# tianyili2017/HEVC-Complexity-Reduction

Measured on AMD Instinct MI355X. Metric: CTUs/sec (ETH-CNN inference), higher is better.
Workload: dtype f32; 1 GPU; All-Intra 3840x2160 QP32, 50 frames synthetic YUV; width=3840, height=2160, frames_per_gpu=50, qp=32, ranks=1, devices_visible=1, rank0_device=0, one_rank_per_device=True, device=AMD Radeon Graphics (gfx950:sramecc+:xnack-, 256 CUs), host NUMA node 1

## Files before the change

### hevc-complexity-reduction_amd/csrc/ethcnn_context.cpp

```cpp
#include "ethcnn_ctx.h"

static thread_local std::string g_create_err;

int set_err(ethcnn_ctx* c, int code, const char* fmt, ...) {
    char buf[512];
    va_list ap;
    va_start(ap, fmt);
    std::vsnprintf(buf, sizeof buf, fmt, ap);
    va_end(ap);
    if (c) c->err = buf; else g_create_err = buf;
    return code;
}

extern "C" const char* ethcnn_version(void) { return "ethcnn-mi355x 0.1 (gfx950)"; }

extern "C" const char* ethcnn_last_error(const ethcnn_ctx* ctx) {
    return ctx ? ctx->err.c_str() : g_create_err.c_str();
}

int ensure_side_streams(ethcnn_ctx* c) {
    hipStream_t* ss[] = {&c->copy_in, &c->copy_out, &c->s_tile};
    for (hipStream_t* s : ss)
        if (!*s) HIPCHK(c, hipStreamCreateWithFlags(s, hipStreamNonBlocking));
    return 0;
}

static void free_workspace(ethcnn_ctx* c) {
    Workspace& w = c->ws;
    void* ptrs[] = {w.featb, w.xs, w.xm, w.xl, w.feat, w.h1, w.h2, w.logits, w.raw, w.flags, c->xs1, c->xm1, c->xl1, c->h1_1, c->flags1};
    for (void* p : ptrs)
        if (p) (void)hipFree(p);
    w = Workspace();
    c->xs1 = c->xm1 = c->xl1 = nullptr;
    c->h1_1 = nullptr;
    c->flags1 = nullptr;
}

Workspace ws_view(const ethcnn_ctx* c, int p) {
// ... 188 lines not shown
    {
        std::vector<std::thread> th;
        for (ethcnn_ctx* p : c->peers)
            if (p) th.emplace_back([p] { ethcnn_destroy(p); });
        for (auto& t : th) t.join();
        c->peers.clear();
    }
    (void)hipSetDevice(c->device);
    for (const auto& r : c->pinned) (void)hipHostFree(const_cast<char*>(r.first));
    delete c->pool;
    if (c->dw_arena) (void)hipFree(c->dw_arena);
    if (c->dw_fast) (void)hipFree(c->dw_fast);
    if (c->dw_trunk16) (void)hipFree(c->dw_trunk16);
    if (c->dw_heads16) (void)hipFree(c->dw_heads16);
    {
        void* lp[] = {c->d_lstm, c->d_vec, c->d_state[0], c->d_state[1], c->d_lprobs, c->d_lgate, c->d_ssync, c->seq_vec, c->seq_probs, c->narrow_buf, c->d_compare};
        for (void* p : lp)
            if (p) (void)hipFree(p);
    }
    {
        hipEvent_t evs[] = {c->e_tile[0], c->e_tile[1], c->e_trunk[0], c->e_trunk[1], c->e_main, c->e_fc1[0], c->e_fc1[1], c->e_band[0], c->e_band[1], c->e_band[2], c->e_band[3]};
        for (hipEvent_t e : evs)
            if (e) (void)hipEventDestroy(e);
    }
    hipStream_t streams[] = {c->stream, c->copy_in, c->copy_out, c->s_tile};
    for (hipStream_t st : streams)
        if (st) (void)hipStreamDestroy(st);
    delete c;
}

extern "C" int ethcnn_get_startup_times(const ethcnn_ctx* c, double* runtime_init_ms, double* create_ms) {
// ... 182 lines not shown
```

### hevc-complexity-reduction_amd/csrc/ethcnn_ctx.h

```cpp
#pragma once
#include <hip/hip_runtime.h>
#if defined(__SSE2__)
#include <emmintrin.h>
#endif
#include <sched.h>
#include <sys/stat.h>
#include <unistd.h>

#include <algorithm>
#include <cerrno>
#include <cstdarg>
#include <cstdio>
#include <cstdlib>
#include <cstring>
#include <atomic>
#include <chrono>
#include <condition_variable>
#include <functional>
#include <mutex>
#include <string>
#include <thread>
#include <vector>

#include "ethcnn_kernels.h"
// ... 120 lines not shown
    float* seq_vec = nullptr;
    float* seq_probs = nullptr;
    size_t seq_vec_cap = 0, seq_probs_cap = 0;
    int seq_chunk = 0;
    ethcnn_source_format src_fmt{8, 420};
    uint8_t* narrow_buf = nullptr;
    size_t narrow_cap = 0;
    int narrow_chunk = 0;
    std::vector<uint8_t> narrow_host;

    Workspace ws;
    uint4 *xs1 = nullptr, *xm1 = nullptr, *xl1 = nullptr;
    float* h1_1 = nullptr;
    int* flags1 = nullptr;
    hipStream_t s_tile = nullptr;
    hipEvent_t e_tile[2] = {}, e_trunk[2] = {}, e_main = nullptr;
    hipEvent_t e_fc1[2] = {};
    int tile_after_fc1 = 0;
    hipEvent_t e_band[4] = {};
    int* d_lgate = nullptr;
    int lgate_chunks = 0;
    bool lgate_clean = false;
    int lgate_n = -1;
    int lstm_epoch = 0;
    int lstm_one_launch = 1;
    int tile_blocks = 256;
    unsigned pass_idx = 0;
    int last_parity = 0;
    int small_launch = 1;
    bool luma_over_pcie = false;
// ... 144 lines not shown
```

### hevc-complexity-reduction_amd/csrc/ethcnn_dense.hip

```cpp
#include <hip/hip_runtime.h>

#include <cstdlib>

#include "ethcnn_kernels.h"
#include "ethcnn_fc1_regs.h"
#include "ethcnn_fc1_tile.h"

namespace ethcnn {

template <int MS, int NS, int WM, int NSUB, bool GROUP, int NST = 3>
__global__ __launch_bounds__(64 * WM) void k_fc1_p3(const float* __restrict__ feat, const float* __restrict__ Wimg,
                                                    const float* __restrict__ bias, float* __restrict__ out, int M) {
    __shared__ __attribute__((aligned(16))) float smem[Fc1Shape<MS, NS, WM, NSUB, NST>::LDS_FLOATS];
    fc1_tile<MS, NS, WM, NSUB, GROUP, NST>(smem, feat, Wimg, bias, out, M, blockIdx.x);
}

#ifdef FC1_STAMPS
__device__ unsigned long long g_fc1_stamps[1 << 14][2];
__device__ __forceinline__ void fc1_stamp(int slot) {
    unsigned long long t;
    asm volatile("s_memrealtime %0\n\ts_waitcnt lgkmcnt(0)" : "=s"(t)::"memory");
    if (threadIdx.x == 0) g_fc1_stamps[blockIdx.x & 0x3fff][slot] = t;
}
#define FC1_STAMP(i) fc1_stamp(i)
#else
#define FC1_STAMP(i)
#endif

#ifndef FC1_BULK_NST
#define FC1_BULK_NST 3
#endif
template <int NS, int WM, int NSUB>
__global__ __launch_bounds__(64 * WM) void k_fc1_bulk(const float* __restrict__ feat, const float* __restrict__ Wimg,
                                                      const float* __restrict__ bias, float* __restrict__ out, int m_main,
                                                      int m_total, unsigned rem_blocks) {
    __shared__ __attribute__((aligned(16))) float smem[Fc1Shape<2, NS, WM, NSUB, FC1_BULK_NST>::LDS_FLOATS];
    FC1_STAMP(0);
    if (blockIdx.x < rem_blocks)
        fc1_tile<1, NS, WM, NSUB, true, FC1_BULK_NST>(smem, feat + (size_t)(m_main / 16) * kNFeat * 16, Wimg, bias, out + (size_t)m_main * kNVec,
                                           m_total - m_main, blockIdx.x);
    else
        fc1_tile<2, NS, WM, NSUB, true, FC1_BULK_NST>(smem, feat, Wimg, bias, out, m_main, blockIdx.x - rem_blocks);
    FC1_STAMP(1);
}

template <int MS, int NS, int WM, int NSUB, bool GROUP = false, int NST = 3>
static void launch_fc1_p3(const float* feat, const float* wimg, const float* bias, float* out, int M, hipStream_t s) {
    constexpr int BM = 16 * MS * WM, NSPLIT = kNVec / (16 * NS);
    const int mtiles = (M + BM - 1) / BM;
    const int blocks = GROUP ? ((mtiles + 7) / 8) * 8 * NSPLIT : mtiles * NSPLIT;
    hipLaunchKernelGGL((k_fc1_p3<MS, NS, WM, NSUB, GROUP, NST>), dim3(blocks), dim3(64 * WM), 0, s, feat, wimg, bias, out, M);
}

template <int NS, int D>
__global__ __launch_bounds__(256) void k_fc1_regs(const float* __restrict__ feat, const float* __restrict__ wlane,
                                                  const float* __restrict__ bias, float* __restrict__ out, int M) {
    int mt, nb;
    fc1_block_to_tile<kNVec / (16 * NS), true>(blockIdx.x, mt, nb);
    if (mt * 64 >= M) return;
    fc1_tile_regs<NS, D, false>(feat, wlane, bias, out, M, mt, nb);
}
template <int NS, int D>
static void launch_fc1_regs(const float* feat, const float* wlane, const float* bias, float* out, int M, hipStream_t s) {
    constexpr int NSPLIT = kNVec / (16 * NS);
    const int mtiles = (M + 63) / 64;
    hipLaunchKernelGGL((k_fc1_regs<NS, D>), dim3(((mtiles + 7) / 8) * 8 * NSPLIT), dim3(256), 0, s, feat, wlane, bias, out, M);
// ... 20 lines not shown
    double tbest = 1e30;
    for (const Shape& sh : shapes) {
        const int blocks = ((n + sh.bm - 1) / sh.bm) * sh.nsplit;
        const double t = sh.a + sh.b * ((blocks + 255) / 256);
        if (t < tbest) { tbest = t; best = sh.variant; }
    }
    return best;
}

static void launch_fc1_rows(int variant, const Workspace& ws, const DeviceWeights& w, int row0, int rows, float* out,
                            hipStream_t s) {
    const float* feat = ws.feat + (size_t)(row0 / 16) * kNFeat * 16;
    float* o = out + (size_t)row0 * kNVec;
    switch (variant) {
        default:
            launch_fc1_p3<2, 7, 4, 1, true>(feat, w.fc1_img112, w.fc1_b, o, rows, s);
            break;
        case 1:
            launch_fc1_p3<1, 7, 4, 1, true>(feat, w.fc1_img112, w.fc1_b, o, rows, s);
            break;
        case 2:
            launch_fc1_p3<1, 4, 4, 2, true>(feat, w.fc1_img64, w.fc1_b, o, rows, s);
            break;
        case 3:
            launch_fc1_p3<1, 2, 4, 2, true>(feat, w.fc1_img32, w.fc1_b, o, rows, s);
            break;
        case 4:
            launch_fc1_p3<1, 1, 4, 4, true>(feat, w.fc1_img16, w.fc1_b, o, rows, s);
            break;
        case 5:
            launch_fc1_p3<1, 2, 4, 4, true>(feat, w.fc1_img32, w.fc1_b, o, rows, s);
            break;
        case 6:
            launch_fc1_p3<1, 2, 2, 4, true>(feat, w.fc1_img32, w.fc1_b, o, rows, s);
            break;
        case 7: launch_fc1_regs<1, 16>(feat, w.fc1_lane16, w.fc1_b, o, rows, s); break;
        case 8: launch_fc1_regs<2, 10>(feat, w.fc1_lane16, w.fc1_b, o, rows, s); break;
        case 9: launch_fc1_regs<4, 6>(feat, w.fc1_lane16, w.fc1_b, o, rows, s); break;
        case 10: launch_fc1_p3<2, 7, 4, 1, false>(feat, w.fc1_img112, w.fc1_b, o, rows, s); break;
        case 11: launch_fc1_p3<1, 7, 4, 1, false>(feat, w.fc1_img112, w.fc1_b, o, rows, s); break;
        case 12: launch_fc1_p3<1, 4, 4, 2, false>(feat, w.fc1_img64, w.fc1_b, o, rows, s); break;
    }
}

void launch_fc1(const Workspace& ws, const DeviceWeights& w, int n, float* out, hipStream_t s) {
    const int variant = fc1_variant();
    if (variant >= 100) {
        const int bt = ((n / 128) * 4 / 256) * 256 / 4;
        if (bt > 0) launch_fc1_rows(0, ws, w, 0, bt * 128, out, s);
        if (n > bt * 128) launch_fc1_rows(variant - 100, ws, w, bt * 128, n - bt * 128, out, s);
        return;
    }
    if (variant >= 0 && variant != 20 && variant != 30) {
        launch_fc1_rows(variant, ws, w, 0, n, out, s);
        return;
    }
    if (variant == 20) {
        launch_fc1_rows(fc1_short_variant(n), ws, w, 0, n, out, s);
        return;
    }
    const int big_tiles = ((n / 128) * 4 / 256) * 256 / 4;
    const int row0 = big_tiles * 128;
    if (big_tiles >= 3 * 192 && n > row0 && fc1_variant() != 30) {
        const int rem_tiles = (n - row0 + 63) / 64;
        const unsigned rem_blocks = (unsigned)((rem_tiles + 7) / 8) * 8 * 4;
        const unsigned main_blocks = (unsigned)((big_tiles + 7) / 8) * 8 * 4;
        hipLaunchKernelGGL((k_fc1_bulk<7, 4, 1>), dim3(rem_blocks + main_blocks), dim3(256), 0, s, ws.feat, w.fc1_img112, w.fc1_b, out,
                           row0, n, rem_blocks);
        return;
    }
    if (big_tiles > 0) launch_fc1_rows(0, ws, w, 0, row0, out, s);
    if (n > row0) launch_fc1_rows(fc1_short_variant(n - row0), ws, w, row0, n - row0, out, s);
}

}
```

### hevc-complexity-reduction_amd/csrc/ethcnn_fc1_tile.h

```cpp
#pragma once
#include <hip/hip_runtime.h>

#include "ethcnn_kernels.h"

namespace ethcnn {

typedef float f32x4 __attribute__((ext_vector_type(4)));
typedef __attribute__((address_space(3))) void lds_void;
typedef const __attribute__((address_space(1))) void glb_void;
#ifndef MFMA16
#define MFMA16(a, b, c) __builtin_amdgcn_mfma_f32_16x16x4f32((a), (b), (c), 0, 0, 0)
#endif
constexpr int kAuxSc1 = 16;

template <int N>
__device__ __forceinline__ void vm_wait() { asm volatile("s_waitcnt vmcnt(%0)" ::"n"(N) : "memory"); }
template <int ISSUE, int MAXK>
__device__ __forceinline__ void vm_wait_groups(int keep) {
    if constexpr (MAXK == 0) {
        vm_wait<0>();
    } else {
        if (keep >= MAXK) vm_wait<MAXK * ISSUE>();
        else vm_wait_groups<ISSUE, MAXK - 1>(keep);
    }
// ... 6 lines not shown
    static constexpr int LDS_FLOATS = NST * STAGE;
};

template <int NSPLIT, bool GROUP>
__device__ __forceinline__ void fc1_block_to_tile(unsigned bid, int& mt, int& nb) {
    if (GROUP) {
        const int xcd = bid & 7, slot = bid >> 3;
        nb = slot % NSPLIT;
        mt = (slot / NSPLIT) * 8 + xcd;
    } else {
        nb = (int)(bid % NSPLIT);
        mt = (int)(bid / NSPLIT);
    }
}

template <int MS, int NS, int WM, int NSUB, int NST, bool COHERENT = false, bool A_SC1 = false>
__device__ __forceinline__ void fc1_tile_at(float* __restrict__ smem, const float* __restrict__ feat, const float* __restrict__ Wimg,
                                            const float* __restrict__ bias, float* __restrict__ out, int M, const int mt, const int nb) {
    constexpr int BK = 16 * NSUB, BN = 16 * NS, BM = 16 * MS * WM;
    constexpr int NK = kNFeat / BK;
    constexpr int B_FLOATS = BK * BN;
    constexpr bool COLSWZ = (BN % 32 == 0);
    constexpr int B_INST = B_FLOATS / 256;
    constexpr int B_PER = (B_INST + WM - 1) / WM;
    constexpr int A_PER = NSUB * MS;
    constexpr int ISSUE = B_PER + A_PER;
    constexpr int A_FLOATS = WM * A_PER * 256;
    constexpr int STAGE = B_FLOATS + A_FLOATS;
    constexpr int DIST = NST - 1;
    static_assert(NK % NST == 0 && NK >= NST, "K chunks must come in whole rounds of the stage ring");
    static_assert(DIST * ISSUE <= 63, "vmcnt is a 6-bit counter");
    static_assert(STAGE == Fc1Shape<MS, NS, WM, NSUB, NST>::STAGE, "LDS budget of the shape");

    const int lane = threadIdx.x & 63, wv = threadIdx.x >> 6;
    const int col = lane & 15, g = lane >> 4;
    const int m0 = mt * BM + wv * 16 * MS;
    const int n0 = nb * BN;

    f32x4 acc[MS][NS];
#pragma unroll
    for (int i = 0; i < MS; ++i)
#pragma unroll
        for (int j = 0; j < NS; ++j) acc[i][j] = (f32x4){0.f, 0.f, 0.f, 0.f};

    const int ngroups = (M + 15) >> 4;
    const unsigned wvu = __builtin_amdgcn_readfirstlane(wv);
    const unsigned lane16 = (unsigned)lane * 16u;
    const int mg0 = __builtin_amdgcn_readfirstlane(m0 >> 4);
    const float* a_base[MS];
#pragma unroll
    for (int i = 0; i < MS; ++i) a_base[i] = feat + (size_t)min(mg0 + i, ngroups - 1) * (kNFeat / 4) * 64;
    const float* b_base[B_PER];
    unsigned b_dst[B_PER];
#pragma unroll
    for (int i = 0; i < B_PER; ++i) {
        const unsigned piece = min(wvu + i * WM, (unsigned)(B_INST - 1));
        b_base[i] = Wimg + (size_t)nb * NK * B_FLOATS + (size_t)piece * 256;
        b_dst[i] = piece * 1024u;
    }
    int bcol[NS];
#pragma unroll
    for (int j = 0; j < NS; ++j) bcol[j] = (j * 16 + col) ^ (COLSWZ ? ((g & 1) << 4) : 0);
    int brow[4];
#pragma unroll
    for (int e = 0; e < 4; ++e) brow[e] = (COLSWZ ? e : (e ^ (g & 1))) * BN;
    float* a_lds = smem + B_FLOATS + wv * A_PER * 256;

    const unsigned lds_base = __builtin_amdgcn_readfirstlane((unsigned)(size_t)(lds_void*)smem);
    const unsigned a_dst0 = lds_base + 4u * (B_FLOATS + wvu * A_PER * 256);
#define P3_DMA(sbase, lds_byte_addr)                                                                   \
    {                                                                                                  \
        unsigned keep_;                                                                                \
        asm volatile("s_mov_b32 %0, m0\n\ts_mov_b32 m0, %3\n\ts_nop 0\n\tglobal_load_lds_dwordx4 %1, %2\n\ts_mov_b32 m0, %0" \
                     : "=&s"(keep_) : "v"(lane16), "s"(sbase), "s"(lds_byte_addr) : "memory");          \
    }
#define P3_DMA_SC1(sbase, lds_byte_addr)                                                               \
    {                                                                                                  \
        unsigned keep_;                                                                                \
        asm volatile("s_mov_b32 %0, m0\n\ts_mov_b32 m0, %3\n\ts_nop 0\n\tglobal_load_lds_dwordx4 %1, %2 sc1\n\ts_mov_b32 m0, %0" \
                     : "=&s"(keep_) : "v"(lane16), "s"(sbase), "s"(lds_byte_addr) : "memory");          \
    }
#define P3_ISSUE(kc, st)                                                                               \
    {                                                                                                  \
        _Pragma("unroll") for (int i = 0; i < B_PER; ++i)                                              \
            P3_DMA(b_base[i] + (size_t)(kc) * B_FLOATS, lds_base + 4u * (st) * STAGE + b_dst[i]);      \
        _Pragma("unroll") for (int u = 0; u < NSUB; ++u)                                               \
            _Pragma("unroll") for (int i = 0; i < MS; ++i) {                                           \
                if (A_SC1) P3_DMA_SC1(a_base[i] + ((size_t)(kc) * NSUB + u) * 256,                     \
                                      a_dst0 + 4u * ((st) * STAGE + (u * MS + i) * 256))               \
                else P3_DMA(a_base[i] + ((size_t)(kc) * NSUB + u) * 256,                               \
                            a_dst0 + 4u * ((st) * STAGE + (u * MS + i) * 256))                         \
            }                                                                                          \
    }
#define P3_COMPUTE(st)                                                                                 \
    {                                                                                                  \
        _Pragma("unroll") for (int u = 0; u < NSUB; ++u) {                                             \
            float4 av[MS];                                                                             \
            _Pragma("unroll") for (int i = 0; i < MS; ++i)                                             \
                av[i] = *reinterpret_cast<const float4*>(a_lds + (st) * STAGE + (u * MS + i) * 256 + lane * 4); \
            const float* bs = smem + (st) * STAGE + (16 * u + 4 * g) * BN;                             \
            _Pragma("unroll") for (int e = 0; e < 4; ++e) {                                            \
                float b[NS];                                                                           \
                _Pragma("unroll") for (int j = 0; j < NS; ++j) b[j] = bs[brow[e] + bcol[j]];           \
                _Pragma("unroll") for (int i = 0; i < MS; ++i) {                                       \
                    const float a = (e == 0) ? av[i].x : (e == 1) ? av[i].y : (e == 2) ? av[i].z : av[i].w; \
                    _Pragma("unroll") for (int j = 0; j < NS; ++j) acc[i][j] = MFMA16(a, b[j], acc[i][j]); \
                }                                                                                      \
            }                                                                                          \
        }                                                                                              \
    }
#define P3_STEP(kc, st)                                                                                \
    {                                                                                                  \
        if ((kc) + DIST < NK) { P3_ISSUE((kc) + DIST, ((st) + DIST) % NST); }                          \
        P3_COMPUTE(st);                                                                                \
        vm_wait_groups<ISSUE, DIST - 1>(NK - 2 - (kc));                                                \
        asm volatile("s_waitcnt lgkmcnt(0)" ::: "memory");                                             \
        __builtin_amdgcn_s_barrier();                                                                  \
    }

    __builtin_amdgcn_s_setprio(2);
#pragma unroll
// ... 14 lines not shown
    const int lane_out = ((m0 + 4 * g) * kNVec + col) * 4;
#pragma unroll
    for (int j = 0; j < NS; ++j) {
        const float bv = bias[n0 + j * 16 + col];
#pragma unroll
        for (int i = 0; i < MS; ++i)
#pragma unroll
            for (int r = 0; r < 4; ++r) {
                const float h = acc[i][j][r] + bv;
                __builtin_amdgcn_raw_buffer_store_b32(__builtin_bit_cast(unsigned, fmaxf(0.2f * h, h)), rO,
                                                      lane_out + (i * 16 + r) * kNVec * 4, (n0 + j * 16) * 4, COHERENT ? kAuxSc1 : 0);
            }
    }
}

template <int MS, int NS, int WM, int NSUB, bool GROUP, int NST>
__device__ __forceinline__ void fc1_tile(float* __restrict__ smem, const float* __restrict__ feat, const float* __restrict__ Wimg,
                                         const float* __restrict__ bias, float* __restrict__ out, int M, const unsigned bid) {
    int mt, nb;
    fc1_block_to_tile<kNVec / (16 * NS), GROUP>(bid, mt, nb);
    if (mt * (16 * MS * WM) >= M) return;
    fc1_tile_at<MS, NS, WM, NSUB, NST>(smem, feat, Wimg, bias, out, M, mt, nb);
}


}
```

### hevc-complexity-reduction_amd/csrc/ethcnn_kernels.h

```cpp
#pragma once
#include <hip/hip_runtime.h>

#include "ethcnn_spec.h"

namespace ethcnn {

struct Workspace {
    int cap = 0;
    uint4* xs = nullptr;
    uint4* xm = nullptr;
    uint4* xl = nullptr;
    float* feat = nullptr;
    uint16_t* featb = nullptr;
    float* h1 = nullptr;
    float* h2 = nullptr;
    float* logits = nullptr;
    float* raw = nullptr;
    int* flags = nullptr;
    int flags_cap = 0;
};

struct FrameGeom {
    int width, height;
    long pitch, frame_stride;
    int cw, ch, nctu;
};

void launch_tile(const uint8_t* d_luma, const FrameGeom& g, long ctu0, int n, const Workspace& ws, int n_flags,
                 hipStream_t s, int max_blocks = 0, const unsigned* wait_rows = nullptr, unsigned wait_seq = 0, unsigned* gave_up = nullptr);
void launch_trunk(const Workspace& ws, const DeviceWeights& w, int n, bool resi, hipStream_t s, int fc1_plan = 0);
void launch_trunk_f16(const Workspace& ws, const DeviceWeights& w, int n, hipStream_t s);
void launch_trunk_f16_foldall(const uint8_t* d_luma, const FrameGeom& g, long ctu0, int n, const Workspace& ws, const DeviceWeights& w, int n_flags,
                              hipStream_t s);
void launch_fc1(const Workspace& ws, const DeviceWeights& w, int n, float* out, hipStream_t s);
void launch_fc1_fast(const Workspace& ws, const DeviceWeights& w, int n, float* out, int plan, hipStream_t s, int cus = 256);
void launch_heads(const Workspace& ws, const DeviceWeights& w, int n, float qn, int nctu_per_frame,
                  long ctu0, float thr1, float thr2, float* d_probs, hipStream_t s);
void launch_heads_f16(const Workspace& ws, const DeviceWeights& w, int n, float qn, int nctu_per_frame, long ctu0, float thr1, float thr2,
                      float* d_probs, hipStream_t s);
#ifdef ETHCNN_FULL_FENCE
#define ETHCNN_HANDOFF_RELEASE() asm volatile("buffer_wbl2 sc1\n\ts_waitcnt vmcnt(0) lgkmcnt(0)" ::: "memory")
#define ETHCNN_HANDOFF_ACQUIRE() asm volatile("buffer_inv sc1" ::: "memory")
#else
#define ETHCNN_HANDOFF_RELEASE() asm volatile("s_waitcnt vmcnt(0)" ::: "memory")
// ... 53 lines not shown
```

### hevc-complexity-reduction_amd/csrc/ethcnn_kernels.hip

```cpp
#include <hip/hip_runtime.h>

#include <cstdlib>

#include "ethcnn_kernels.h"

namespace ethcnn {

int chunks_per_frame(int nctu) { return (nctu + kSubBatch - 1) / kSubBatch; }


__global__ __launch_bounds__(256) void k5_gate(float* __restrict__ probs, const int* __restrict__ flags, int N,
                                               GateIndex gi, float thr2) {
    const int idx = blockIdx.x * 256 + threadIdx.x;
    const int i = idx / kNOut, j = idx % kNOut;
    if (i >= N || j == 0) return;
    const int chunk = gate_chunk(gi, i);
    const bool open32 = flags[2 * chunk] != 0;
    const bool open16 = open32 ? (flags[2 * chunk + 1] != 0) : (0.0f > thr2);
    if (j < 5 ? !open32 : !open16) probs[(size_t)i * kNOut + j] = 0.0f;
}

void launch_gate(const Workspace& ws, int n, int nctu, long ctu0, float thr2, float* d_probs, hipStream_t s) {
    const long total = (long)n * kNOut;
    hipLaunchKernelGGL(k5_gate, dim3((unsigned)((total + 255) / 256)), dim3(256), 0, s, d_probs, ws.flags, n,
                       make_gate_index(nctu, ctu0), thr2);
}

typedef float f32x4_cal __attribute__((ext_vector_type(4)));
__global__ __launch_bounds__(256) void k_mfma_rate(int iters, float* sink) {
    f32x4_cal acc[4] = {{0.f, 0.f, 0.f, 0.f}, {0.f, 0.f, 0.f, 0.f}, {0.f, 0.f, 0.f, 0.f}, {0.f, 0.f, 0.f, 0.f}};
    const float a = 1.0f + threadIdx.x * 1e-7f, b = 0.999f;
    for (int i = 0; i < iters; ++i) {
#pragma unroll
        for (int u = 0; u < 8; ++u)
#pragma unroll
            for (int j = 0; j < 4; ++j) acc[j] = __builtin_amdgcn_mfma_f32_16x16x4f32(a, b, acc[j], 0, 0, 0);
    }
    const float s = acc[0][0] + acc[1][1] + acc[2][2] + acc[3][3];
    if (s == 123.456f) *sink = s;
}
// ... 6 lines not shown
```

### hevc-complexity-reduction_amd/csrc/ethcnn_model.cpp

```cpp
#include "ethcnn_ctx.h"

static int upload_weights(ethcnn_ctx* c) {
    HIPCHK(c, hipSetDevice(c->device));
    std::vector<size_t> sizes = {(size_t)3 * kTrunkWFrags * 64, (size_t)3 * kTrunkBFrags * 64,
                                 (size_t)kNFeat * kNVec, (size_t)kNVec};
    for (int h = 0; h < 3; ++h) { sizes.push_back((size_t)(kN1[h] + 1) * kN2[h]); sizes.push_back((size_t)kN2[h]); }
    for (int h = 0; h < 3; ++h) { sizes.push_back((size_t)(kN2[h] + 1) * kN3[h]); sizes.push_back((size_t)kN3[h]); }
    sizes.push_back((size_t)kNFeat * kNVec);
    sizes.push_back((size_t)kNFeat * kNVec);
    sizes.push_back((size_t)kNFeat * kNVec);
    sizes.push_back((size_t)kNFeat * kNVec);
    for (int h = 0; h < 3; ++h) sizes.push_back((size_t)kN1[h] * kN2[h]);
    std::vector<size_t> offs;
    size_t total = 0;
    for (size_t s : sizes) { offs.push_back(total); total += (s + 63) / 64 * 64; }
    std::vector<float> host(total, 0.0f);
    const float* blob = c->blob.data();
    pack_trunk_fragments(blob, host.data() + offs[0], host.data() + offs[1]);
    {
        std::vector<float> wcat((size_t)kNFeat * kNVec);
        pack_fc1(blob, wcat.data(), host.data() + offs[3]);
        pack_fc1_image(wcat.data(), 112, 16, host.data() + offs[2]);
        pack_fc1_image(wcat.data(), 64, 32, host.data() + offs[16]);
        pack_fc1_image(wcat.data(), 32, 32, host.data() + offs[17]);
        pack_fc1_image(wcat.data(), 16, 32, host.data() + offs[18]);
        pack_fc1_lane_image(wcat.data(), host.data() + offs[19]);
    }
    for (int h = 0; h < 3; ++h) {
        std::memcpy(host.data() + offs[4 + 2 * h], blob + kOffFc2W[h], sizes[4 + 2 * h] * 4);
        std::memcpy(host.data() + offs[5 + 2 * h], blob + kOffFc2B[h], sizes[5 + 2 * h] * 4);
        std::memcpy(host.data() + offs[10 + 2 * h], blob + kOffFc3W[h], sizes[10 + 2 * h] * 4);
        std::memcpy(host.data() + offs[11 + 2 * h], blob + kOffFc3B[h], sizes[11 + 2 * h] * 4);
        pack_fc2_lane_image(blob + kOffFc2W[h], kN1[h], kN2[h], host.data() + offs[20 + h]);
    }
    if (!c->dw_arena) HIPCHK(c, hipMalloc((void**)&c->dw_arena, total * 4));
    HIPCHK(c, hipDeviceSynchronize());
    HIPCHK(c, hipMemcpy(c->dw_arena, host.data(), total * 4, hipMemcpyHostToDevice));
    DeviceWeights& d = c->dw;
    d.trunk_w = c->dw_arena + offs[0];
    d.trunk_b = c->dw_arena + offs[1];
    d.fc1_img112 = c->dw_arena + offs[2];
    d.fc1_img64 = c->dw_arena + offs[16];
    d.fc1_img32 = c->dw_arena + offs[17];
    d.fc1_img16 = c->dw_arena + offs[18];
    d.fc1_lane16 = c->dw_arena + offs[19];
    for (int h = 0; h < 3; ++h) d.fc2_lane[h] = c->dw_arena + offs[20 + h];
    d.fc1_b = c->dw_arena + offs[3];
    for (int h = 0; h < 3; ++h) {
        d.fc2_w[h] = c->dw_arena + offs[4 + 2 * h];
        d.fc2_b[h] = c->dw_arena + offs[5 + 2 * h];
        d.fc3_w[h] = c->dw_arena + offs[10 + 2 * h];
        d.fc3_b[h] = c->dw_arena + offs[11 + 2 * h];
    }
    d.fc1_fast = nullptr;
    d.trunk16_w = nullptr;
    d.heads16_w = nullptr;
    d.trunk16_c = nullptr;
    c->guard_state[2] = c->guard_state[3] = 0;
    ++c->weights_gen;
    c->have_weights = true;
    return ETHCNN_OK;
// ... 280 lines not shown
```

### hevc-complexity-reduction_amd/csrc/ethcnn_pass.cpp

```cpp
#include "ethcnn_ctx.h"

int make_geom(ethcnn_ctx* c, int w, int h, ptrdiff_t pitch, ptrdiff_t fstride, FrameGeom* g) {
    if (w <= 0 || h <= 0) return set_err(c, ETHCNN_ERR_ARG, "bad frame size %dx%d", w, h);
    if (pitch < w) return set_err(c, ETHCNN_ERR_ARG, "pitch %td < width %d", pitch, w);
    g->width = w;
    g->height = h;
    g->pitch = (long)pitch;
    g->frame_stride = (long)fstride;
    g->cw = (w + 63) / 64;
    g->ch = (h + 63) / 64;
    g->nctu = g->cw * g->ch;
    return 0;
}

unsigned done_arm(ethcnn_ctx* c) {
    if (!c->done_sync || !c->h_done) return 0;
    if (++c->done_seq == 0) ++c->done_seq;
    return c->done_seq;
}
hipError_t stream_sync(ethcnn_ctx* c) {
    const unsigned seq = c->done_armed;
    c->done_armed = 0;
    if (seq) {
        const auto t0 = std::chrono::steady_clock::now();
// ... 49 lines not shown
    const int cpf = chunks_per_frame(g.nctu);
    const long nchunks = (ctu0 + n - 1) / g.nctu * cpf + ((ctu0 + n - 1) % g.nctu) / kSubBatch + 1 -
                         (ctu0 / g.nctu * cpf + (ctu0 % g.nctu) / kSubBatch);
    c->done_armed = 0;
    const bool takes_small = c->small_launch && n < kPipelineMinCtus && small_pass_ok(d_luma, g, n);
    int rc = (c->fc1_plan && !takes_small) ? ensure_fast_weights(c, c->fc1_plan) : 0;
    if (rc) return rc;
    rc = ensure_workspace(c, n, (int)nchunks);
    if (rc) return rc;
    const float qn = (float)qp * (1.0f / 51.0f);
    const int fast = c->fc1_plan;
    const bool foldall = fast == 3 && c->tile_wait_rows == nullptr;
    const bool side_tile = c->overlap != 0 && n >= kPipelineMinCtus && !foldall;
    const int p = side_tile ? (int)(c->pass_idx++ & 1) : 0;
    const Workspace w = ws_view(c, p);
    if (side_tile && !c->s_tile && (rc = ensure_side_streams(c)) != 0) return rc;
    hipStream_t s_tile = side_tile ? c->s_tile : c->stream;
    if (input_ready) HIPCHK(c, hipStreamWaitEvent(s_tile, input_ready, 0));
    Workspace wv = w;
    if (!c->debug_capture) wv.h2 = wv.logits = wv.raw = nullptr;
    const bool small = !side_tile && c->small_launch && small_pass_ok(d_luma, g, n);
    if (small) {
        rc = run_small_pass(c, d_luma, g, ctu0, n, false, wv, w.h1, qn, d_probs_pass, (int)nchunks, c->luma_over_pcie,
                            c->luma_over_pcie ? c->tile_wait_rows : nullptr);
        if (rc) return rc;
    } else {
        if (side_tile) {
            HIPCHK(c, hipStreamWaitEvent(s_tile, c->e_trunk[p], 0));
            if (c->main_dirty) {
                HIPCHK(c, hipEventRecord(c->e_main, c->stream));
                c->main_dirty = false;
            }
            HIPCHK(c, hipStreamWaitEvent(s_tile, c->e_main, 0));
            const bool behind_fc1 = c->tile_after_fc1 != 0 && fast != 0;
            HIPCHK(c, hipStreamWaitEvent(s_tile, behind_fc1 ? c->e_fc1[p ^ 1] : c->e_trunk[p ^ 1], 0));
        }
        (void)hipGetLastError();
#define LAUNCH_OK(name)                                                                                            \
    do {                                                                                                           \
        const hipError_t le_ = hipGetLastError();                                                                  \
        if (le_ != hipSuccess) return set_err(c, ETHCNN_ERR_DEVICE, "launch of the %s stage failed: %s", name, hipGetErrorString(le_)); \
    } while (0)
        if (!foldall) {
            StageTimer t(c, ETHCNN_STAGE_TILE, n, s_tile);
            launch_tile(d_luma, g, ctu0, n, w, sync_words((int)nchunks), s_tile, side_tile ? c->tile_blocks : 0,
                        side_tile ? nullptr : c->tile_wait_rows, c->rows_seq, c->h_done + 1);
        }
        LAUNCH_OK("tile");
        if (side_tile) {
            HIPCHK(c, hipEventRecord(c->e_tile[p], s_tile));
            HIPCHK(c, hipStreamWaitEvent(c->stream, c->e_tile[p], 0));
        }
        {
            StageTimer t(c, ETHCNN_STAGE_TRUNK);
            if (foldall) launch_trunk_f16_foldall(d_luma, g, ctu0, n, w, c->dw, sync_words((int)nchunks), c->stream);
            else if (fast == 3) launch_trunk_f16(w, c->dw, n, c->stream);
            else launch_trunk(w, c->dw, n, false, c->stream, fast);
        }
        LAUNCH_OK("trunk");
        if (side_tile) HIPCHK(c, hipEventRecord(c->e_trunk[p], c->stream));
        if (fast) {
// ... 129 lines not shown
```

### hevc-complexity-reduction_amd/csrc/ethcnn_spec.h

```cpp
#pragma once
#include <cstddef>
#include <cstdint>
#include <cstdlib>

#include "../../include/ethcnn.h"

namespace ethcnn {

#ifdef ETHCNN_EXPERIMENTS
inline const char* dev_env(const char* name) { return std::getenv(name); }
#else
inline const char* dev_env(const char*) { return nullptr; }
#endif

constexpr int kCtu = 64;
constexpr int kNOut = 21;
constexpr int kNFeat = 2688;
constexpr int kNVec = 448;
constexpr int kNFc2 = 336;
constexpr int kSubBatch = 1024;
constexpr size_t kBlobFloats = 1288210;
constexpr int kMaxCtusPerPass = 131072;
static_assert((long long)(kMaxCtusPerPass / 16) * kNFeat * 16 * 4 < (1ll << 31), "trunk: group image byte offset must fit int32");
static_assert((long long)kMaxCtusPerPass * kNVec * 4 < (1ll << 31), "FC1 / heads: h1 byte offsets must fit int32");
// ... 125 lines not shown
};
constexpr double kFastGuardTol = 2.5e-5;
FastGuard fast_plan_floor_bound(const float* blob, int plan, bool heads16);

constexpr int kOff3[3] = {0, 512, 640};
constexpr int kOff2[3] = {672, 2208, 2592};
constexpr int kNb[3] = {4, 2, 1};

constexpr int kTrunkWFrags = 84, kTrunkBFrags = 20;
constexpr int kTrunkResiTabAt = kTrunkWFrags * 64 + 8 * 64 * 4;
constexpr int kTrunkResiLds = kTrunkResiTabAt + 4096;

struct DeviceWeights {
    float* trunk_w = nullptr;
    float* trunk_b = nullptr;
    float* fc1_img112 = nullptr;
    float* fc1_img64 = nullptr;
    float* fc1_img32 = nullptr;
    float* fc1_img16 = nullptr;
    float* fc1_lane16 = nullptr;
    uint16_t* fc1_fast = nullptr;
    uint16_t* trunk16_w = nullptr;
    float* trunk16_c = nullptr;
    Trunk16Scalars trunk16_s{};
    uint16_t* heads16_w = nullptr;
    Heads16Scalars heads16_s{};
    float fast_scale_a = 1.0f, fast_scale_w = 1.0f;
    float* fc1_b = nullptr;
    float* fc2_w[3] = {nullptr, nullptr, nullptr};
    float* fc2_b[3] = {nullptr, nullptr, nullptr};
    float* fc2_lane[3] = {nullptr, nullptr, nullptr};
// ... 27 lines not shown
```

### hevc-complexity-reduction_amd/csrc/ethcnn_tile.hip

```cpp
#include <hip/hip_runtime.h>

#include "ethcnn_kernels.h"
#include "ethcnn_tile_group.h"

namespace ethcnn {

template <bool FAST, bool WAIT>
__global__ __launch_bounds__(256) void k0_tile_slab(const uint8_t* __restrict__ luma, int width, int height, long pitch,
                                                    long frame_stride, int cw, int nctu, long ctu0, int n_total,
                                                    uint4* __restrict__ XS, uint4* __restrict__ XM,
                                                    uint4* __restrict__ XL, int* __restrict__ gate_flags, int n_flags, TileWait tw) {
    __shared__ uint32_t tile[16 * kSlabCtuPitch];
    if (blockIdx.x == 0)
        for (int i = threadIdx.x; i < n_flags; i += 256) gate_flags[i] = 0;
    const int ngroups = (n_total + 15) >> 4;
#pragma unroll 1
    for (int grp = blockIdx.x; grp < ngroups; grp += gridDim.x) {
        if (WAIT) tile_wait_rows(tw, ctu0, grp, n_total, nctu, cw);
        tile_group<FAST, false, false>(tile, luma, width, height, pitch, frame_stride, cw, nctu, ctu0, n_total, grp, XS, XM, XL);
    }
}

void launch_tile(const uint8_t* d_luma, const FrameGeom& g, long ctu0, int n, const Workspace& ws, int n_flags,
                 hipStream_t s, int max_blocks, const unsigned* wait_rows, unsigned wait_seq, unsigned* gave_up) {
    const int blocks = (n + 15) / 16;
    const bool fast = (g.width % 16 == 0) && (g.pitch % 16 == 0) && (g.frame_stride % 16 == 0) &&
                      (reinterpret_cast<uintptr_t>(d_luma) % 16 == 0);
    const int sb = max_blocks > 0 ? (blocks < max_blocks ? blocks : max_blocks) : blocks;
    const TileWait tw{wait_rows, wait_seq, gave_up};
    if (wait_rows && fast)
        hipLaunchKernelGGL((k0_tile_slab<true, true>), dim3(sb), dim3(256), 0, s, d_luma, g.width, g.height, g.pitch,
                           g.frame_stride, g.cw, g.nctu, ctu0, n, ws.xs, ws.xm, ws.xl, ws.flags, n_flags, tw);
    else if (wait_rows)
        hipLaunchKernelGGL((k0_tile_slab<false, true>), dim3(sb), dim3(256), 0, s, d_luma, g.width, g.height, g.pitch,
                           g.frame_stride, g.cw, g.nctu, ctu0, n, ws.xs, ws.xm, ws.xl, ws.flags, n_flags, tw);
// ... 10 lines not shown
```

Before: 41.74 million CTU/s.

## Use lane-ordered FC1 weight image, dynamic tile ticketing, per-chunk gate kernel

The FC1 MFMA tile kernels now read a lane-ordered weight image, so each lane loads one float4 per column tile from LDS instead of doing scattered scalar LDS reads. The 112-wide image is dropped and its arena slot reused. The side-stream tiling kernel now hands out work groups dynamically through an atomic ticket counter instead of a fixed grid stride, which balances load across blocks. The gate kernel launches one block per chunk and only zeroes closed ranges instead of one thread per output element. These add an atomic per group, with the ticket reset relying on the last drawer, and a new weight-packing path that must match the kernel indexing.

```diff
diff --git a/hevc-complexity-reduction_amd/csrc/ethcnn_context.cpp b/hevc-complexity-reduction_amd/csrc/ethcnn_context.cpp
--- a/hevc-complexity-reduction_amd/csrc/ethcnn_context.cpp
+++ b/hevc-complexity-reduction_amd/csrc/ethcnn_context.cpp
@@ -22,6 +22,10 @@
     hipStream_t* ss[] = {&c->copy_in, &c->copy_out, &c->s_tile};
     for (hipStream_t* s : ss)
         if (!*s) HIPCHK(c, hipStreamCreateWithFlags(s, hipStreamNonBlocking));
+    if (!c->d_tile_ticket) {
+        HIPCHK(c, hipMalloc((void**)&c->d_tile_ticket, 64));
+        HIPCHK(c, hipMemsetAsync(c->d_tile_ticket, 0, 64, c->s_tile));
+    }
     return 0;
 }
 
@@ -240,7 +244,7 @@
     if (c->dw_trunk16) (void)hipFree(c->dw_trunk16);
     if (c->dw_heads16) (void)hipFree(c->dw_heads16);
     {
-        void* lp[] = {c->d_lstm, c->d_vec, c->d_state[0], c->d_state[1], c->d_lprobs, c->d_lgate, c->d_ssync, c->seq_vec, c->seq_probs, c->narrow_buf, c->d_compare};
+        void* lp[] = {c->d_lstm, c->d_vec, c->d_state[0], c->d_state[1], c->d_lprobs, c->d_lgate, c->d_ssync, c->d_tile_ticket, c->seq_vec, c->seq_probs, c->narrow_buf, c->d_compare};
         for (void* p : lp)
             if (p) (void)hipFree(p);
     }
diff --git a/hevc-complexity-reduction_amd/csrc/ethcnn_ctx.h b/hevc-complexity-reduction_amd/csrc/ethcnn_ctx.h
--- a/hevc-complexity-reduction_amd/csrc/ethcnn_ctx.h
+++ b/hevc-complexity-reduction_amd/csrc/ethcnn_ctx.h
@@ -158,6 +158,7 @@
     float* h1_1 = nullptr;
     int* flags1 = nullptr;
     hipStream_t s_tile = nullptr;
+    int* d_tile_ticket = nullptr;
     hipEvent_t e_tile[2] = {}, e_trunk[2] = {}, e_main = nullptr;
     hipEvent_t e_fc1[2] = {};
     int tile_after_fc1 = 0;
diff --git a/hevc-complexity-reduction_amd/csrc/ethcnn_dense.hip b/hevc-complexity-reduction_amd/csrc/ethcnn_dense.hip
--- a/hevc-complexity-reduction_amd/csrc/ethcnn_dense.hip
+++ b/hevc-complexity-reduction_amd/csrc/ethcnn_dense.hip
@@ -8,11 +8,11 @@
 
 namespace ethcnn {
 
-template <int MS, int NS, int WM, int NSUB, bool GROUP, int NST = 3>
+template <int MS, int NS, int WM, int NSUB, bool GROUP, int NST = 3, bool LANE16 = false>
 __global__ __launch_bounds__(64 * WM) void k_fc1_p3(const float* __restrict__ feat, const float* __restrict__ Wimg,
                                                     const float* __restrict__ bias, float* __restrict__ out, int M) {
     __shared__ __attribute__((aligned(16))) float smem[Fc1Shape<MS, NS, WM, NSUB, NST>::LDS_FLOATS];
-    fc1_tile<MS, NS, WM, NSUB, GROUP, NST>(smem, feat, Wimg, bias, out, M, blockIdx.x);
+    fc1_tile<MS, NS, WM, NSUB, GROUP, NST, LANE16>(smem, feat, Wimg, bias, out, M, blockIdx.x);
 }
 
 #ifdef FC1_STAMPS
@@ -37,19 +37,19 @@
     __shared__ __attribute__((aligned(16))) float smem[Fc1Shape<2, NS, WM, NSUB, FC1_BULK_NST>::LDS_FLOATS];
     FC1_STAMP(0);
     if (blockIdx.x < rem_blocks)
-        fc1_tile<1, NS, WM, NSUB, true, FC1_BULK_NST>(smem, feat + (size_t)(m_main / 16) * kNFeat * 16, Wimg, bias, out + (size_t)m_main * kNVec,
+        fc1_tile<1, NS, WM, NSUB, true, FC1_BULK_NST, true>(smem, feat + (size_t)(m_main / 16) * kNFeat * 16, Wimg, bias, out + (size_t)m_main * kNVec,
                                            m_total - m_main, blockIdx.x);
     else
-        fc1_tile<2, NS, WM, NSUB, true, FC1_BULK_NST>(smem, feat, Wimg, bias, out, m_main, blockIdx.x - rem_blocks);
+        fc1_tile<2, NS, WM, NSUB, true, FC1_BULK_NST, true>(smem, feat, Wimg, bias, out, m_main, blockIdx.x - rem_blocks);
     FC1_STAMP(1);
 }
 
-template <int MS, int NS, int WM, int NSUB, bool GROUP = false, int NST = 3>
+template <int MS, int NS, int WM, int NSUB, bool GROUP = false, int NST = 3, bool LANE16 = false>
 static void launch_fc1_p3(const float* feat, const float* wimg, const float* bias, float* out, int M, hipStream_t s) {
     constexpr int BM = 16 * MS * WM, NSPLIT = kNVec / (16 * NS);
     const int mtiles = (M + BM - 1) / BM;
     const int blocks = GROUP ? ((mtiles + 7) / 8) * 8 * NSPLIT : mtiles * NSPLIT;
-    hipLaunchKernelGGL((k_fc1_p3<MS, NS, WM, NSUB, GROUP, NST>), dim3(blocks), dim3(64 * WM), 0, s, feat, wimg, bias, out, M);
+    hipLaunchKernelGGL((k_fc1_p3<MS, NS, WM, NSUB, GROUP, NST, LANE16>), dim3(blocks), dim3(64 * WM), 0, s, feat, wimg, bias, out, M);
 }
 
 template <int NS, int D>
@@ -100,10 +100,10 @@
     float* o = out + (size_t)row0 * kNVec;
     switch (variant) {
         default:
-            launch_fc1_p3<2, 7, 4, 1, true>(feat, w.fc1_img112, w.fc1_b, o, rows, s);
+            launch_fc1_p3<2, 7, 4, 1, true, 3, true>(feat, w.fc1_lane16, w.fc1_b, o, rows, s);
             break;
         case 1:
-            launch_fc1_p3<1, 7, 4, 1, true>(feat, w.fc1_img112, w.fc1_b, o, rows, s);
+            launch_fc1_p3<1, 7, 4, 1, true, 3, true>(feat, w.fc1_lane16, w.fc1_b, o, rows, s);
             break;
         case 2:
             launch_fc1_p3<1, 4, 4, 2, true>(feat, w.fc1_img64, w.fc1_b, o, rows, s);
@@ -123,8 +123,8 @@
         case 7: launch_fc1_regs<1, 16>(feat, w.fc1_lane16, w.fc1_b, o, rows, s); break;
         case 8: launch_fc1_regs<2, 10>(feat, w.fc1_lane16, w.fc1_b, o, rows, s); break;
         case 9: launch_fc1_regs<4, 6>(feat, w.fc1_lane16, w.fc1_b, o, rows, s); break;
-        case 10: launch_fc1_p3<2, 7, 4, 1, false>(feat, w.fc1_img112, w.fc1_b, o, rows, s); break;
-        case 11: launch_fc1_p3<1, 7, 4, 1, false>(feat, w.fc1_img112, w.fc1_b, o, rows, s); break;
+        case 10: launch_fc1_p3<2, 7, 4, 1, false, 3, true>(feat, w.fc1_lane16, w.fc1_b, o, rows, s); break;
+        case 11: launch_fc1_p3<1, 7, 4, 1, false, 3, true>(feat, w.fc1_lane16, w.fc1_b, o, rows, s); break;
         case 12: launch_fc1_p3<1, 4, 4, 2, false>(feat, w.fc1_img64, w.fc1_b, o, rows, s); break;
     }
 }
@@ -151,7 +151,7 @@
         const int rem_tiles = (n - row0 + 63) / 64;
         const unsigned rem_blocks = (unsigned)((rem_tiles + 7) / 8) * 8 * 4;
         const unsigned main_blocks = (unsigned)((big_tiles + 7) / 8) * 8 * 4;
-        hipLaunchKernelGGL((k_fc1_bulk<7, 4, 1>), dim3(rem_blocks + main_blocks), dim3(256), 0, s, ws.feat, w.fc1_img112, w.fc1_b, out,
+        hipLaunchKernelGGL((k_fc1_bulk<7, 4, 1>), dim3(rem_blocks + main_blocks), dim3(256), 0, s, ws.feat, w.fc1_lane16, w.fc1_b, out,
                            row0, n, rem_blocks);
         return;
     }
diff --git a/hevc-complexity-reduction_amd/csrc/ethcnn_fc1_tile.h b/hevc-complexity-reduction_amd/csrc/ethcnn_fc1_tile.h
--- a/hevc-complexity-reduction_amd/csrc/ethcnn_fc1_tile.h
+++ b/hevc-complexity-reduction_amd/csrc/ethcnn_fc1_tile.h
@@ -44,7 +44,10 @@
     }
 }
 
-template <int MS, int NS, int WM, int NSUB, int NST, bool COHERENT = false, bool A_SC1 = false>
+#ifndef FC1_LANE16_JSTEP
+#define FC1_LANE16_JSTEP 2
+#endif
+template <int MS, int NS, int WM, int NSUB, int NST, bool COHERENT = false, bool A_SC1 = false, bool LANE16 = false>
 __device__ __forceinline__ void fc1_tile_at(float* __restrict__ smem, const float* __restrict__ feat, const float* __restrict__ Wimg,
                                             const float* __restrict__ bias, float* __restrict__ out, int M, const int mt, const int nb) {
     constexpr int BK = 16 * NSUB, BN = 16 * NS, BM = 16 * MS * WM;
@@ -61,6 +64,9 @@
     static_assert(NK % NST == 0 && NK >= NST, "K chunks must come in whole rounds of the stage ring");
     static_assert(DIST * ISSUE <= 63, "vmcnt is a 6-bit counter");
     static_assert(STAGE == Fc1Shape<MS, NS, WM, NSUB, NST>::STAGE, "LDS budget of the shape");
+    static_assert(!LANE16 || (NSUB == 1 && B_INST == NS), "the lane image is read per 16-k sub-chunk: one piece per column tile");
+    constexpr int B_ADV = LANE16 ? 256 : B_FLOATS;
+    constexpr int LANE16_JSTEP = FC1_LANE16_JSTEP;
 
     const int lane = threadIdx.x & 63, wv = threadIdx.x >> 6;
     const int col = lane & 15, g = lane >> 4;
@@ -85,7 +91,8 @@
 #pragma unroll
     for (int i = 0; i < B_PER; ++i) {
         const unsigned piece = min(wvu + i * WM, (unsigned)(B_INST - 1));
-        b_base[i] = Wimg + (size_t)nb * NK * B_FLOATS + (size_t)piece * 256;
+        b_base[i] = LANE16 ? Wimg + (size_t)(nb * NS + piece) * (kNFeat / 16) * 256
+                           : Wimg + (size_t)nb * NK * B_FLOATS + (size_t)piece * 256;
         b_dst[i] = piece * 1024u;
     }
     int bcol[NS];
@@ -113,7 +120,7 @@
 #define P3_ISSUE(kc, st)                                                                               \
     {                                                                                                  \
         _Pragma("unroll") for (int i = 0; i < B_PER; ++i)                                              \
-            P3_DMA(b_base[i] + (size_t)(kc) * B_FLOATS, lds_base + 4u * (st) * STAGE + b_dst[i]);      \
+            P3_DMA(b_base[i] + (size_t)(kc) * B_ADV, lds_base + 4u * (st) * STAGE + b_dst[i]);      \
         _Pragma("unroll") for (int u = 0; u < NSUB; ++u)                                               \
             _Pragma("unroll") for (int i = 0; i < MS; ++i) {                                           \
                 if (A_SC1) P3_DMA_SC1(a_base[i] + ((size_t)(kc) * NSUB + u) * 256,                     \
@@ -128,13 +135,26 @@
             float4 av[MS];                                                                             \
             _Pragma("unroll") for (int i = 0; i < MS; ++i)                                             \
                 av[i] = *reinterpret_cast<const float4*>(a_lds + (st) * STAGE + (u * MS + i) * 256 + lane * 4); \
-            const float* bs = smem + (st) * STAGE + (16 * u + 4 * g) * BN;                             \
-            _Pragma("unroll") for (int e = 0; e < 4; ++e) {                                            \
-                float b[NS];                                                                           \
-                _Pragma("unroll") for (int j = 0; j < NS; ++j) b[j] = bs[brow[e] + bcol[j]];           \
-                _Pragma("unroll") for (int i = 0; i < MS; ++i) {                                       \
-                    const float a = (e == 0) ? av[i].x : (e == 1) ? av[i].y : (e == 2) ? av[i].z : av[i].w; \
-                    _Pragma("unroll") for (int j = 0; j < NS; ++j) acc[i][j] = MFMA16(a, b[j], acc[i][j]); \
+            if constexpr (LANE16) {                                                                    \
+                f32x4 b[NS];                                                                           \
+                _Pragma("unroll") for (int j = 0; j < NS; ++j)                                         \
+                    b[j] = *reinterpret_cast<const f32x4*>(smem + (st) * STAGE + j * 256 + lane * 4);  \
+                _Pragma("unroll") for (int j0 = 0; j0 < NS; j0 += LANE16_JSTEP)                        \
+                    _Pragma("unroll") for (int e = 0; e < 4; ++e)                                      \
+                        _Pragma("unroll") for (int i = 0; i < MS; ++i) {                               \
+                            const float a = (e == 0) ? av[i].x : (e == 1) ? av[i].y : (e == 2) ? av[i].z : av[i].w; \
+                            _Pragma("unroll") for (int j = j0; j < j0 + LANE16_JSTEP && j < NS; ++j)   \
+                                acc[i][j] = MFMA16(a, b[j][e], acc[i][j]);                             \
+                        }                                                                              \
+            } else {                                                                                   \
+                const float* bs = smem + (st) * STAGE + (16 * u + 4 * g) * BN;                         \
+                _Pragma("unroll") for (int e = 0; e < 4; ++e) {                                        \
+                    float b[NS];                                                                       \
+                    _Pragma("unroll") for (int j = 0; j < NS; ++j) b[j] = bs[brow[e] + bcol[j]];       \
+                    _Pragma("unroll") for (int i = 0; i < MS; ++i) {                                   \
+                        const float a = (e == 0) ? av[i].x : (e == 1) ? av[i].y : (e == 2) ? av[i].z : av[i].w; \
+                        _Pragma("unroll") for (int j = 0; j < NS; ++j) acc[i][j] = MFMA16(a, b[j], acc[i][j]); \
+                    }                                                                                  \
                 }                                                                                      \
             }                                                                                          \
         }                                                                                              \
@@ -179,14 +199,14 @@
     }
 }
 
-template <int MS, int NS, int WM, int NSUB, bool GROUP, int NST>
+template <int MS, int NS, int WM, int NSUB, bool GROUP, int NST, bool LANE16 = false>
 __device__ __forceinline__ void fc1_tile(float* __restrict__ smem, const float* __restrict__ feat, const float* __restrict__ Wimg,
                                          const float* __restrict__ bias, float* __restrict__ out, int M, const unsigned bid) {
     int mt, nb;
     fc1_block_to_tile<kNVec / (16 * NS), GROUP>(bid, mt, nb);
     if (mt * (16 * MS * WM) >= M) return;
-    fc1_tile_at<MS, NS, WM, NSUB, NST>(smem, feat, Wimg, bias, out, M, mt, nb);
-}
-
-
-}
+    fc1_tile_at<MS, NS, WM, NSUB, NST, false, false, LANE16>(smem, feat, Wimg, bias, out, M, mt, nb);
+}
+
+
+}
diff --git a/hevc-complexity-reduction_amd/csrc/ethcnn_kernels.h b/hevc-complexity-reduction_amd/csrc/ethcnn_kernels.h
--- a/hevc-complexity-reduction_amd/csrc/ethcnn_kernels.h
+++ b/hevc-complexity-reduction_amd/csrc/ethcnn_kernels.h
@@ -28,6 +28,8 @@
 
 void launch_tile(const uint8_t* d_luma, const FrameGeom& g, long ctu0, int n, const Workspace& ws, int n_flags,
                  hipStream_t s, int max_blocks = 0, const unsigned* wait_rows = nullptr, unsigned wait_seq = 0, unsigned* gave_up = nullptr);
+void launch_tile_side(const uint8_t* d_luma, const FrameGeom& g, long ctu0, int n, const Workspace& ws, int n_flags,
+                      hipStream_t s, int max_blocks, int* ticket);
 void launch_trunk(const Workspace& ws, const DeviceWeights& w, int n, bool resi, hipStream_t s, int fc1_plan = 0);
 void launch_trunk_f16(const Workspace& ws, const DeviceWeights& w, int n, hipStream_t s);
 void launch_trunk_f16_foldall(const uint8_t* d_luma, const FrameGeom& g, long ctu0, int n, const Workspace& ws, const DeviceWeights& w, int n_flags,
diff --git a/hevc-complexity-reduction_amd/csrc/ethcnn_kernels.hip b/hevc-complexity-reduction_amd/csrc/ethcnn_kernels.hip
--- a/hevc-complexity-reduction_amd/csrc/ethcnn_kernels.hip
+++ b/hevc-complexity-reduction_amd/csrc/ethcnn_kernels.hip
@@ -11,19 +11,24 @@
 
 __global__ __launch_bounds__(256) void k5_gate(float* __restrict__ probs, const int* __restrict__ flags, int N,
                                                GateIndex gi, float thr2) {
-    const int idx = blockIdx.x * 256 + threadIdx.x;
-    const int i = idx / kNOut, j = idx % kNOut;
-    if (i >= N || j == 0) return;
-    const int chunk = gate_chunk(gi, i);
+    const int chunk = blockIdx.x;
     const bool open32 = flags[2 * chunk] != 0;
     const bool open16 = open32 ? (flags[2 * chunk + 1] != 0) : (0.0f > thr2);
-    if (j < 5 ? !open32 : !open16) probs[(size_t)i * kNOut + j] = 0.0f;
+    if (open32 && open16) return;
+    const int c = chunk + gi.c0, f = c / gi.cpf, k = c - f * gi.cpf;
+    const int rows = min(kSubBatch, gi.nctu - k * kSubBatch);
+    const int i0 = f * gi.nctu + k * kSubBatch - gi.r0;
+    const int i1 = min(i0 + rows, N);
+    const int j0 = open32 ? 5 : 1, nj = (open16 ? 5 : kNOut) - j0;
+    if (nj <= 0) return;
+    for (int t = threadIdx.x; t < (i1 - i0) * nj; t += 256) probs[(size_t)(i0 + t / nj) * kNOut + j0 + t % nj] = 0.0f;
 }
 
 void launch_gate(const Workspace& ws, int n, int nctu, long ctu0, float thr2, float* d_probs, hipStream_t s) {
-    const long total = (long)n * kNOut;
-    hipLaunchKernelGGL(k5_gate, dim3((unsigned)((total + 255) / 256)), dim3(256), 0, s, d_probs, ws.flags, n,
-                       make_gate_index(nctu, ctu0), thr2);
+    const GateIndex gi = make_gate_index(nctu, ctu0);
+    const long last = gi.r0 + (long)n - 1;
+    const int nchunks = (int)(last / nctu) * gi.cpf + (int)(last % nctu) / kSubBatch - gi.c0 + 1;
+    hipLaunchKernelGGL(k5_gate, dim3((unsigned)nchunks), dim3(256), 0, s, d_probs, ws.flags, n, gi, thr2);
 }
 
 typedef float f32x4_cal __attribute__((ext_vector_type(4)));
diff --git a/hevc-complexity-reduction_amd/csrc/ethcnn_model.cpp b/hevc-complexity-reduction_amd/csrc/ethcnn_model.cpp
--- a/hevc-complexity-reduction_amd/csrc/ethcnn_model.cpp
+++ b/hevc-complexity-reduction_amd/csrc/ethcnn_model.cpp
@@ -3,10 +3,9 @@
 static int upload_weights(ethcnn_ctx* c) {
     HIPCHK(c, hipSetDevice(c->device));
     std::vector<size_t> sizes = {(size_t)3 * kTrunkWFrags * 64, (size_t)3 * kTrunkBFrags * 64,
-                                 (size_t)kNFeat * kNVec, (size_t)kNVec};
+                                 (size_t)kNFeat * kNVec , (size_t)kNVec};
     for (int h = 0; h < 3; ++h) { sizes.push_back((size_t)(kN1[h] + 1) * kN2[h]); sizes.push_back((size_t)kN2[h]); }
     for (int h = 0; h < 3; ++h) { sizes.push_back((size_t)(kN2[h] + 1) * kN3[h]); sizes.push_back((size_t)kN3[h]); }
-    sizes.push_back((size_t)kNFeat * kNVec);
     sizes.push_back((size_t)kNFeat * kNVec);
     sizes.push_back((size_t)kNFeat * kNVec);
     sizes.push_back((size_t)kNFeat * kNVec);
@@ -20,18 +19,17 @@
     {
         std::vector<float> wcat((size_t)kNFeat * kNVec);
         pack_fc1(blob, wcat.data(), host.data() + offs[3]);
-        pack_fc1_image(wcat.data(), 112, 16, host.data() + offs[2]);
+        pack_fc1_lane_image(wcat.data(), host.data() + offs[2]);
         pack_fc1_image(wcat.data(), 64, 32, host.data() + offs[16]);
         pack_fc1_image(wcat.data(), 32, 32, host.data() + offs[17]);
         pack_fc1_image(wcat.data(), 16, 32, host.data() + offs[18]);
-        pack_fc1_lane_image(wcat.data(), host.data() + offs[19]);
     }
     for (int h = 0; h < 3; ++h) {
         std::memcpy(host.data() + offs[4 + 2 * h], blob + kOffFc2W[h], sizes[4 + 2 * h] * 4);
         std::memcpy(host.data() + offs[5 + 2 * h], blob + kOffFc2B[h], sizes[5 + 2 * h] * 4);
         std::memcpy(host.data() + offs[10 + 2 * h], blob + kOffFc3W[h], sizes[10 + 2 * h] * 4);
         std::memcpy(host.data() + offs[11 + 2 * h], blob + kOffFc3B[h], sizes[11 + 2 * h] * 4);
-        pack_fc2_lane_image(blob + kOffFc2W[h], kN1[h], kN2[h], host.data() + offs[20 + h]);
+        pack_fc2_lane_image(blob + kOffFc2W[h], kN1[h], kN2[h], host.data() + offs[19 + h]);
     }
     if (!c->dw_arena) HIPCHK(c, hipMalloc((void**)&c->dw_arena, total * 4));
     HIPCHK(c, hipDeviceSynchronize());
@@ -39,12 +37,11 @@
     DeviceWeights& d = c->dw;
     d.trunk_w = c->dw_arena + offs[0];
     d.trunk_b = c->dw_arena + offs[1];
-    d.fc1_img112 = c->dw_arena + offs[2];
     d.fc1_img64 = c->dw_arena + offs[16];
     d.fc1_img32 = c->dw_arena + offs[17];
     d.fc1_img16 = c->dw_arena + offs[18];
-    d.fc1_lane16 = c->dw_arena + offs[19];
-    for (int h = 0; h < 3; ++h) d.fc2_lane[h] = c->dw_arena + offs[20 + h];
+    d.fc1_lane16 = c->dw_arena + offs[2];
+    for (int h = 0; h < 3; ++h) d.fc2_lane[h] = c->dw_arena + offs[19 + h];
     d.fc1_b = c->dw_arena + offs[3];
     for (int h = 0; h < 3; ++h) {
         d.fc2_w[h] = c->dw_arena + offs[4 + 2 * h];
diff --git a/hevc-complexity-reduction_amd/csrc/ethcnn_pass.cpp b/hevc-complexity-reduction_amd/csrc/ethcnn_pass.cpp
--- a/hevc-complexity-reduction_amd/csrc/ethcnn_pass.cpp
+++ b/hevc-complexity-reduction_amd/csrc/ethcnn_pass.cpp
@@ -87,7 +87,7 @@
     const bool side_tile = c->overlap != 0 && n >= kPipelineMinCtus && !foldall;
     const int p = side_tile ? (int)(c->pass_idx++ & 1) : 0;
     const Workspace w = ws_view(c, p);
-    if (side_tile && !c->s_tile && (rc = ensure_side_streams(c)) != 0) return rc;
+    if (side_tile && (!c->s_tile || !c->d_tile_ticket) && (rc = ensure_side_streams(c)) != 0) return rc;
     hipStream_t s_tile = side_tile ? c->s_tile : c->stream;
     if (input_ready) HIPCHK(c, hipStreamWaitEvent(s_tile, input_ready, 0));
     Workspace wv = w;
@@ -116,8 +116,8 @@
     } while (0)
         if (!foldall) {
             StageTimer t(c, ETHCNN_STAGE_TILE, n, s_tile);
-            launch_tile(d_luma, g, ctu0, n, w, sync_words((int)nchunks), s_tile, side_tile ? c->tile_blocks : 0,
-                        side_tile ? nullptr : c->tile_wait_rows, c->rows_seq, c->h_done + 1);
+            if (side_tile) launch_tile_side(d_luma, g, ctu0, n, w, sync_words((int)nchunks), s_tile, c->tile_blocks, c->d_tile_ticket);
+            else launch_tile(d_luma, g, ctu0, n, w, sync_words((int)nchunks), s_tile, 0, c->tile_wait_rows, c->rows_seq, c->h_done + 1);
         }
         LAUNCH_OK("tile");
         if (side_tile) {
diff --git a/hevc-complexity-reduction_amd/csrc/ethcnn_spec.h b/hevc-complexity-reduction_amd/csrc/ethcnn_spec.h
--- a/hevc-complexity-reduction_amd/csrc/ethcnn_spec.h
+++ b/hevc-complexity-reduction_amd/csrc/ethcnn_spec.h
@@ -163,7 +163,6 @@
 struct DeviceWeights {
     float* trunk_w = nullptr;
     float* trunk_b = nullptr;
-    float* fc1_img112 = nullptr;
     float* fc1_img64 = nullptr;
     float* fc1_img32 = nullptr;
     float* fc1_img16 = nullptr;
diff --git a/hevc-complexity-reduction_amd/csrc/ethcnn_tile.hip b/hevc-complexity-reduction_amd/csrc/ethcnn_tile.hip
--- a/hevc-complexity-reduction_amd/csrc/ethcnn_tile.hip
+++ b/hevc-complexity-reduction_amd/csrc/ethcnn_tile.hip
@@ -19,6 +19,47 @@
         if (WAIT) tile_wait_rows(tw, ctu0, grp, n_total, nctu, cw);
         tile_group<FAST, false, false>(tile, luma, width, height, pitch, frame_stride, cw, nctu, ctu0, n_total, grp, XS, XM, XL);
     }
+}
+
+template <bool FAST>
+__global__ __launch_bounds__(256) void k0_tile_side(const uint8_t* __restrict__ luma, int width, int height, long pitch,
+                                                    long frame_stride, int cw, int nctu, long ctu0, int n_total,
+                                                    uint4* __restrict__ XS, uint4* __restrict__ XM,
+                                                    uint4* __restrict__ XL, int* __restrict__ gate_flags, int n_flags,
+                                                    int* __restrict__ ticket) {
+    __shared__ uint32_t tile[16 * kSlabCtuPitch];
+    __shared__ int s_draw;
+    if (blockIdx.x == 0)
+        for (int i = threadIdx.x; i < n_flags; i += 256) gate_flags[i] = 0;
+    const int ngroups = (n_total + 15) >> 4;
+    int grp = blockIdx.x;
+#pragma unroll 1
+    for (;;) {
+        tile_group<FAST, false, false>(tile, luma, width, height, pitch, frame_stride, cw, nctu, ctu0, n_total, grp, XS, XM, XL);
+        if (threadIdx.x == 0) s_draw = __hip_atomic_fetch_add(ticket, 1, __ATOMIC_RELAXED, __HIP_MEMORY_SCOPE_AGENT);
+        __syncthreads();
+        const int draw = s_draw;
+        __syncthreads();
+        grp = (int)gridDim.x + draw;
+        if (grp >= ngroups) {
+            if (threadIdx.x == 0 && draw == ngroups - 1) __hip_atomic_store(ticket, 0, __ATOMIC_RELAXED, __HIP_MEMORY_SCOPE_AGENT);
+            break;
+        }
+    }
+}
+
+void launch_tile_side(const uint8_t* d_luma, const FrameGeom& g, long ctu0, int n, const Workspace& ws, int n_flags,
+                      hipStream_t s, int max_blocks, int* ticket) {
+    const int groups = (n + 15) / 16;
+    const int sb = groups < max_blocks ? groups : max_blocks;
+    const bool fast = (g.width % 16 == 0) && (g.pitch % 16 == 0) && (g.frame_stride % 16 == 0) &&
+                      (reinterpret_cast<uintptr_t>(d_luma) % 16 == 0);
+    if (fast)
+        hipLaunchKernelGGL((k0_tile_side<true>), dim3(sb), dim3(256), 0, s, d_luma, g.width, g.height, g.pitch,
+                           g.frame_stride, g.cw, g.nctu, ctu0, n, ws.xs, ws.xm, ws.xl, ws.flags, n_flags, ticket);
+    else
+        hipLaunchKernelGGL((k0_tile_side<false>), dim3(sb), dim3(256), 0, s, d_luma, g.width, g.height, g.pitch,
+                           g.frame_stride, g.cw, g.nctu, ctu0, n, ws.xs, ws.xm, ws.xl, ws.flags, n_flags, ticket);
 }
 
 void launch_tile(const uint8_t* d_luma, const FrameGeom& g, long ctu0, int n, const Workspace& ws, int n_flags,
```

After: 41.90 million CTU/s, median of 6. Within noise of the previous version (+0.4%).
